# jkulhanek/viewformer

Measured on AMD Instinct MI355X. Metric: novel views/sec (encode->AR transformer->decode), 128px 6-ctx, higher is better.
Workload: dtype bf16

## Files before the change

viewformer_amd/csrc/gemm_bf16_g256.hip:

```cpp
#include "vf_common.h"
#include "epilogue.h"
#include "../../include/vf_hip.h"

namespace {

typedef __bf16 bf16x8 __attribute__((ext_vector_type(8)));
typedef __bf16 bf16x2_t __attribute__((ext_vector_type(2)));

constexpr int GM = 256, GN = 256, GK = 64;
constexpr int GA_BYTES = GM * GK * 2;
constexpr int GB_BYTES = GN * GK * 2;
constexpr int GSTAGE = GA_BYTES + GB_BYTES;

__device__ __forceinline__ void bufds16(__amdgpu_buffer_rsrc_t r, void* l, unsigned voff, unsigned soff) {
    __builtin_amdgcn_raw_ptr_buffer_load_lds(r, (__attribute__((address_space(3))) void*)l, 16, voff, soff, 0, 0);
}

template <bool DROP, int IC>
__device__ __forceinline__ void g256_store_f32(const vf_igemm_args& p, const f32x16 (&acc)[IC][2], int m_tile0, int n_tile0, int wrow0,
                                               int wave_n, int half, int l31, bool full, bool gelu) {
    const long long ldc = p.ldc, ldr = p.ldr;
    const bool has_res = p.res != nullptr;
    const bool dual = p.epilogue == VF_EPI_GELU_DUAL;
    const int odd = l31 & 1;
    const uint32_t drop_thresh = vf_dropout_thresh(p.drop_rate), drop_key = vf_dropout_key(p.drop_seed, p.drop_site, 0u);
    const float drop_scale = 1.0f / (1.0f - p.drop_rate);
#pragma unroll
    for (int j = 0; j < 2; ++j) {
        const int n = n_tile0 + wave_n * 64 + j * 32 + l31;
        const float bias = p.bias ? p.bias[n] : 0.f;
#pragma unroll
        for (int i = 0; i < IC; ++i) {
            int m0 = m_tile0 + wrow0 + i * 32 + 4 * half;
            if constexpr (DROP) asm volatile("" : "+v"(m0) :: "memory");
            const int rows_left = p.M - m0;
            float* o = p.out + (size_t)(rows_left > 0 ? m0 : 0) * ldc + n;
            float v[16];
#pragma unroll
            for (int r = 0; r < 16; ++r) v[r] = acc[i][j][r] + bias;
            if (gelu) {
#pragma unroll
                for (int r = 0; r < 16; ++r) v[r] = vf_gelu_erf_fast(v[r]);
            }
            if constexpr (DROP) {
#pragma unroll
                for (int g = 0; g < 4; ++g) {
                    const uint32_t w = vf_dropout_word(drop_key, (uint32_t)(((m0 + p.drop_row0) >> 2) + 2 * g) * (uint32_t)p.Cout + (uint32_t)n);
#pragma unroll
                    for (int e = 0; e < 4; ++e) v[4 * g + e] = vf_dropout_keep(w, e, drop_thresh) ? v[4 * g + e] * drop_scale : 0.f;
                }
            }
            if (has_res) {
                const float* rs = p.res + (size_t)(rows_left > 0 ? m0 : 0) * ldr + n;
                float rr[16];
#pragma unroll
                for (int r = 0; r < 16; ++r) {
                    const int row = (r & 3) + 8 * (r >> 2);
                    rr[r] = rs[(long long)(full || row < rows_left ? row : 0) * ldr];
                }
#pragma unroll
                for (int r = 0; r < 16; ++r) v[r] += rr[r];
            }
            if (full) {
#pragma unroll
                for (int r = 0; r < 16; ++r) o[(long long)((r & 3) + 8 * (r >> 2)) * ldc] = v[r];
            } else if (rows_left > 0) {
#pragma unroll
                for (int r = 0; r < 16; ++r) {
                    const int row = (r & 3) + 8 * (r >> 2);
                    if (row < rows_left) o[(long long)row * ldc] = v[r];
                }
            }
            if (dual) {
                __builtin_amdgcn_sched_barrier(0);
                __bf16* o16 = reinterpret_cast<__bf16*>(p.out_aux) + (size_t)(rows_left > 0 ? m0 : 0) * ldc + (n - odd);
#pragma unroll
                for (int r = 0; r < 16; ++r) v[r] = vf_gelu_erf_fast(v[r]);
#pragma unroll
                for (int r = 0; r < 16; r += 2) {
                    const float give = odd ? v[r] : v[r + 1];
                    const float got = vf_lane_xor1(give);
                    const int row = ((r + odd) & 3) + 8 * ((r + odd) >> 2);
                    bf16x2_t h;
                    h[0] = (__bf16)(odd ? got : v[r]);
                    h[1] = (__bf16)(odd ? v[r + 1] : got);
                    if (full || row < rows_left) *reinterpret_cast<bf16x2_t*>(o16 + (long long)row * ldc) = h;
                }
            }
            __builtin_amdgcn_sched_barrier(0);
        }
    }
}

template <int EPI, bool FULL, int IC>
__device__ __forceinline__ void g256_store_bf16(const vf_igemm_args& p, const f32x16 (&acc)[IC][2], int m_tile0, int n_tile0, int wrow0,
                                                int wave_n, int half, int l31) {
    __bf16* __restrict__ O = reinterpret_cast<__bf16*>(p.out);
    const int odd = l31 & 1;
#pragma unroll
    for (int j = 0; j < 2; ++j) {
        const int n = n_tile0 + wave_n * 64 + j * 32 + l31;
        const float bias = p.bias ? p.bias[n] : 0.f;
#pragma unroll
        for (int i = 0; i < IC; ++i) {
            const int m0 = m_tile0 + wrow0 + i * 32 + 4 * half;
            float t[16];
            if (EPI == 2 || EPI == 4) {
                const bool u16 = p.reserved0 & 4;
                const unsigned esz = u16 ? 2u : 4u;
                const __amdgpu_buffer_rsrc_t u_rs = __builtin_amdgcn_make_buffer_rsrc(
                    const_cast<unsigned char*>(reinterpret_cast<const unsigned char*>(p.res) + (size_t)m_tile0 * p.ldr * esz), 0,
                    (int)min((long long)0x7fffffff, (long long)(p.M - m_tile0) * p.ldr * esz), 0x00020000);
                float uu[16];
                if (u16) {
                    const unsigned voff = ((unsigned)(m0 - m_tile0) * (unsigned)p.ldr + (unsigned)(n - odd)) * 2u;
                    unsigned w[8];
#pragma unroll
                    for (int r = 0; r < 16; r += 2) {
                        const int row = ((r + odd) & 3) + 8 * ((r + odd) >> 2);
                        w[r >> 1] = __builtin_amdgcn_raw_buffer_load_b32(u_rs, voff + (unsigned)row * (unsigned)p.ldr * 2u, 0, 0);
                    }
#pragma unroll
                    for (int r = 0; r < 16; r += 2) {
                        const unsigned mine = w[r >> 1];
                        const unsigned give = odd ? (mine << 16) : (mine & 0xffff0000u);
                        const unsigned got = vf_lane_xor1(give);
                        uu[r] = __builtin_bit_cast(float, odd ? got : (mine << 16));
                        uu[r + 1] = __builtin_bit_cast(float, odd ? (mine & 0xffff0000u) : got);
                    }
                } else {
                    const unsigned voff = ((unsigned)(m0 - m_tile0) * (unsigned)p.ldr + (unsigned)n) * 4u;
#pragma unroll
                    for (int r = 0; r < 16; ++r) {
                        const unsigned soff = (unsigned)((r & 3) + 8 * (r >> 2)) * (unsigned)p.ldr * 4u;
                        uu[r] = __builtin_bit_cast(float, __builtin_amdgcn_raw_buffer_load_b32(u_rs, voff, soff, 0));
                    }
                }
                __builtin_amdgcn_sched_barrier(0);
#pragma unroll
                for (int q = 0; q < 4; ++q) {
#pragma unroll
                    for (int e = 0; e < 4; ++e)
                        t[4 * q + e] = __fmul_rn(__fadd_rn(acc[i][j][4 * q + e], bias), EPI == 4 ? uu[4 * q + e] : vf_gelu_grad_fast(uu[4 * q + e]));
                    __builtin_amdgcn_sched_barrier(0);
                }
            } else {
#pragma unroll
                for (int r = 0; r < 16; ++r) {
                    t[r] = acc[i][j][r] + bias;
                    if (EPI == 1) t[r] = vf_gelu_erf_fast(t[r]);
                }
            }
            float gq[EPI == 5 ? 16 : 1];
            if (EPI == 5) {
#pragma unroll
                for (int r = 0; r < 16; ++r) { float f, g; vf_gelu_and_grad_fast(t[r], f, g); t[r] = f; gq[r] = g; }
            }
#pragma unroll
            for (int pass = 0; pass < ((EPI == 3 || EPI == 5) ? 2 : 1); ++pass) {
                __bf16* __restrict__ dst = pass == 0 ? O : reinterpret_cast<__bf16*>(p.out_aux);
                if (EPI == 3 && pass == 1) {
                    __builtin_amdgcn_sched_barrier(0);
#pragma unroll
                    for (int r = 0; r < 16; ++r) t[r] = vf_gelu_erf_fast(t[r]);
                }
#pragma unroll
                for (int r = 0; r < 16; r += 2) {
                    const float lo = (EPI == 5 && pass == 0) ? gq[r] : t[r], hi = (EPI == 5 && pass == 0) ? gq[r + 1] : t[r + 1];
                    const float give = odd ? lo : hi;
                    const float got = vf_lane_xor1(give);
                    const int m = m0 + ((r + odd) & 3) + 8 * ((r + odd) >> 2);
                    bf16x2_t v;
                    v[0] = (__bf16)(odd ? got : lo);
                    v[1] = (__bf16)(odd ? hi : got);
                    if (FULL || m < p.M) *reinterpret_cast<bf16x2_t*>(dst + (size_t)m * p.ldc + (n - odd)) = v;
                }
            }
        }
    }
}

template <bool O16, bool DROP, int IC>
__device__ __forceinline__ void g256_tile(const vf_igemm_args& p, unsigned char* smem_b, int m_tile0, int nblk, int tid) {
    constexpr int TROWS = 2 * IC * 32;
    const int lane = tid & 63;
    const int wave = __builtin_amdgcn_readfirstlane(tid >> 6);
    const int wave_m = wave >> 2, wave_n = wave & 3;
    const int half = lane >> 5, l31 = lane & 31;
    const int wrow0 = wave_m * (IC * 32);
    const int n_tile0 = nblk * GN;
    const int nstages = p.Cin / GK;

    const bool a_mover = wave * 32 < TROWS;
    const __amdgpu_buffer_rsrc_t a_rsrc = __builtin_amdgcn_make_buffer_rsrc(const_cast<float*>(p.x), 0, 0x7fffffff, 0x00020000);
    const __amdgpu_buffer_rsrc_t w_rsrc = __builtin_amdgcn_make_buffer_rsrc(const_cast<float*>(p.w_packed), 0, 0x7fffffff, 0x00020000);
    unsigned avoff[4];
#pragma unroll
    for (int q = 0; q < 4; ++q) {
        const int r = wave * 32 + q * 8 + (lane >> 3);
        const int c = (lane & 7) ^ ((r >> 1) & 7);
        int m = m_tile0 + r;
        m = m < p.M ? m : p.M - 1;
        avoff[q] = (unsigned)(((size_t)m * p.lda) * 2 + c * 16);
    }
    const unsigned wvoff = (unsigned)((size_t)nblk * GB_BYTES + wave * 4096 + lane * 16);
    const size_t w_stage_stride = (size_t)(p.Cout / 128) * (GK * 128 * 2);
    auto issue = [&](int s) {
        unsigned char* dst = smem_b + (s & 1) * GSTAGE;
        if (IC == 4 || a_mover) {
#pragma unroll
            for (int q = 0; q < 4; ++q) bufds16(a_rsrc, dst + (wave * 32 + q * 8) * 128, avoff[q], (unsigned)(s * (GK * 2)));
        }
#pragma unroll
        for (int q = 0; q < 4; ++q) bufds16(w_rsrc, dst + GA_BYTES + wave * 4096 + q * 1024, wvoff + q * 1024, (unsigned)((size_t)s * w_stage_stride));
    };

    const unsigned a_row_off = (unsigned)((wrow0 + l31) * 128);
    const unsigned a_swz = (unsigned)((l31 >> 1) & 7);
    unsigned a_off[4];
#pragma unroll
    for (int ks = 0; ks < 4; ++ks) a_off[ks] = a_row_off + ((((unsigned)(ks * 2 + half)) ^ a_swz) << 4);
    const unsigned b_off = (unsigned)(GA_BYTES + (wave_n >> 1) * (GK * 128 * 2) + ((half * 128) + (wave_n & 1) * 64 + l31) * 16);

    f32x16 acc[IC][2];
#pragma unroll
    for (int i = 0; i < IC; ++i)
#pragma unroll
        for (int j = 0; j < 2; ++j)
#pragma unroll
            for (int r = 0; r < 16; ++r) acc[i][j][r] = 0.f;

    issue(0);
    for (int s = 0; s < nstages; ++s) {
        asm volatile("s_waitcnt vmcnt(0) lgkmcnt(0)" ::: "memory");
        __builtin_amdgcn_s_barrier();
        if (s + 1 < nstages) issue(s + 1);
        const unsigned char* buf = smem_b + (s & 1) * GSTAGE;
        bf16x8 a[2][IC], b[2][2];
        auto frags = [&](int ks, bf16x8 (&af)[IC], bf16x8 (&bf)[2]) {
#pragma unroll
            for (int j = 0; j < 2; ++j) bf[j] = *reinterpret_cast<const bf16x8*>(buf + b_off + (ks * 2 * 128 + j * 32) * 16);
#pragma unroll
            for (int i = 0; i < IC; ++i) af[i] = *reinterpret_cast<const bf16x8*>(buf + a_off[ks] + i * (32 * 128));
        };
        frags(0, a[0], b[0]);
#pragma unroll
        for (int ks = 0; ks < 4; ++ks) {
            if (ks < 3) frags(ks + 1, a[(ks + 1) & 1], b[(ks + 1) & 1]);
            __builtin_amdgcn_sched_barrier(0);
#pragma unroll
            for (int i = 0; i < IC; ++i)
#pragma unroll
                for (int j = 0; j < 2; ++j)
                    acc[i][j] = __builtin_amdgcn_mfma_f32_32x32x16_bf16(a[ks & 1][i], b[ks & 1][j], acc[i][j], 0, 0, 0);
            __builtin_amdgcn_sched_barrier(0);
        }
    }

    const bool full = m_tile0 + TROWS <= p.M;
    const bool gelu = p.epilogue == VF_EPI_GELU_ERF;
    if (O16) {
        const bool gbwd = p.epilogue == VF_EPI_GELU_BWD;
        const bool dual16 = p.epilogue == VF_EPI_GELU_DUAL;
        const bool deriv = p.reserved0 & 8;
        if (dual16 && deriv) {
            if (full) g256_store_bf16<5, true, IC>(p, acc, m_tile0, n_tile0, wrow0, wave_n, half, l31);
            else g256_store_bf16<5, false, IC>(p, acc, m_tile0, n_tile0, wrow0, wave_n, half, l31);
        } else if (gbwd && deriv) {
            if (full) g256_store_bf16<4, true, IC>(p, acc, m_tile0, n_tile0, wrow0, wave_n, half, l31);
            else g256_store_bf16<4, false, IC>(p, acc, m_tile0, n_tile0, wrow0, wave_n, half, l31);
        } else if (dual16) {
            if (full) g256_store_bf16<3, true, IC>(p, acc, m_tile0, n_tile0, wrow0, wave_n, half, l31);
            else g256_store_bf16<3, false, IC>(p, acc, m_tile0, n_tile0, wrow0, wave_n, half, l31);
        } else if (full) {
            if (gbwd) g256_store_bf16<2, true, IC>(p, acc, m_tile0, n_tile0, wrow0, wave_n, half, l31);
            else if (gelu) g256_store_bf16<1, true, IC>(p, acc, m_tile0, n_tile0, wrow0, wave_n, half, l31);
            else g256_store_bf16<0, true, IC>(p, acc, m_tile0, n_tile0, wrow0, wave_n, half, l31);
        } else {
            if (gbwd) g256_store_bf16<2, false, IC>(p, acc, m_tile0, n_tile0, wrow0, wave_n, half, l31);
            else if (gelu) g256_store_bf16<1, false, IC>(p, acc, m_tile0, n_tile0, wrow0, wave_n, half, l31);
            else g256_store_bf16<0, false, IC>(p, acc, m_tile0, n_tile0, wrow0, wave_n, half, l31);
        }
    } else {
        g256_store_f32<DROP, IC>(p, acc, m_tile0, n_tile0, wrow0, wave_n, half, l31, full, gelu);
    }
}

__device__ __forceinline__ void g256_panel_order(unsigned lbid, int mt, int nb, int& mtile, int& nblk) {
    constexpr int PANEL = 4;
    const int sn = nb <= PANEL ? nb : nb % PANEL == 0 ? PANEL : nb % 3 == 0 ? 3 : nb % 2 == 0 ? 2 : 1;
    const int per_panel = mt * sn;
    const int panel = (int)(lbid / (unsigned)per_panel);
    const int in_panel = (int)(lbid - (unsigned)panel * per_panel);
    nblk = panel * sn + in_panel % sn;
    mtile = in_panel / sn;
}

template <bool O16, bool DROP = false, bool TAIL = false>
__global__ __launch_bounds__(512, 1) void gemm_bf16_g256_kernel(vf_igemm_args p, int f_rows, int h_rows, int tail_ic) {
    extern __shared__ __attribute__((aligned(16))) unsigned char smem_b[];
    const int tid = threadIdx.x;
    const int nb = p.Cout / GN;
    int mtile, nblk;
    if constexpr (!TAIL) {
        g256_panel_order(vf_xcd_bid(), (p.M + GM - 1) / GM, nb, mtile, nblk);
        g256_tile<O16, DROP, 4>(p, smem_b, mtile * GM, nblk, tid);
    } else {
        const unsigned F = (unsigned)(f_rows * nb), tot = gridDim.x;
        const unsigned x = blockIdx.x & 7u, i = blockIdx.x >> 3;
        const unsigned nF = F / 8u + (x < (F & 7u) ? 1u : 0u);
        const unsigned baseF = x * (F / 8u) + (x < (F & 7u) ? x : (F & 7u));
        if (i < nF) {
            g256_panel_order(baseF + i, f_rows, nb, mtile, nblk);
            g256_tile<O16, DROP, 4>(p, smem_b, mtile * GM, nblk, tid);
            return;
        }
        const unsigned baseT = x * (tot / 8u) + (x < (tot & 7u) ? x : (tot & 7u));
        g256_panel_order(baseT - baseF + (i - nF), h_rows, nb, mtile, nblk);
        const int m_tile0 = f_rows * GM + mtile * (tail_ic * 64);
        if (tail_ic == 3) g256_tile<O16, DROP, 3>(p, smem_b, m_tile0, nblk, tid);
        else g256_tile<O16, DROP, 2>(p, smem_b, m_tile0, nblk, tid);
    }
}

}

struct G256Tail { int f_rows, h_rows, ic; };
static G256Tail g256_tail_policy(int M, int nb) {
    const int mt = (M + GM - 1) / GM;
    const long long ntiles = (long long)mt * nb;
    constexpr int CUS = 256;
    G256Tail none{0, 0, 0};
    if (ntiles <= CUS || !vf_selected(VF_SEL_GEMM_TAIL)) return none;
    const int last = (int)(ntiles % CUS);
    if (last == 0 || last > (CUS * 3) / 4 - 8 || last < 16) return none;
    const int f_rows = (int)((ntiles / CUS) * CUS / nb);
    if (f_rows <= 0 || f_rows >= mt) return none;
    const int rem_blocks = (M - f_rows * GM + 31) / 32;
    for (int ic = 2; ic <= 3; ++ic) {
        const int h_rows = (rem_blocks + 2 * ic - 1) / (2 * ic);
        if ((long long)h_rows * nb <= CUS) return G256Tail{f_rows, h_rows, ic};
    }
    return none;
}

int vf_gemm_bf16_g256_launch(const vf_igemm_args& a, hipStream_t stream) {
    const bool a16 = a.reserved0 & 1, o16 = a.reserved0 & 2;
    if (!a16 || a.batch > 1 || a.Cout % GN != 0 || a.Cin % GK != 0 || a.M < GM || (a.lda & 7)) return VF_ERR_UNSUPPORTED;
    if (o16 && ((a.res && a.epilogue != VF_EPI_GELU_BWD) || (a.ldc & 1))) return VF_ERR_UNSUPPORTED;
    if (a.epilogue == VF_EPI_GELU_BWD && !(o16 && a.res)) return VF_ERR_UNSUPPORTED;
    if (a.epilogue == VF_EPI_GELU_DUAL && (a.res || !a.out_aux || (a.ldc & 1))) return VF_ERR_UNSUPPORTED;
    if ((a.reserved0 & 4) && a.epilogue != VF_EPI_GELU_BWD) return VF_ERR_BAD_ARG;
    if (a.reserved0 & 8) {
        if (a.epilogue == VF_EPI_GELU_BWD ? !(a.reserved0 & 4) : !(a.epilogue == VF_EPI_GELU_DUAL && o16)) return VF_ERR_BAD_ARG;
    }
    if (a.res && a.epilogue == VF_EPI_GELU_ERF) return VF_ERR_UNSUPPORTED;
    if (a.drop_rate != 0.f && (!(a.drop_rate > 0.f && a.drop_rate < 1.f) || o16 || a.epilogue != VF_EPI_NONE || a.drop_row0 < 0 || (a.drop_row0 & 3) ||
                               (((unsigned long long)a.M + (unsigned long long)a.drop_row0 + 3) / 4) * (unsigned long long)a.Cout >= (1ull << 32)))
        return VF_ERR_UNSUPPORTED;
    if ((size_t)a.M * a.lda * 2 >= (1ull << 31) || (size_t)a.Cin * a.Cout * 2 >= (1ull << 31)) return VF_ERR_UNSUPPORTED;
    const int mt = (a.M + GM - 1) / GM, nb = a.Cout / GN;
    const G256Tail t = g256_tail_policy(a.M, nb);
    const dim3 g((unsigned)(t.f_rows ? (t.f_rows + t.h_rows) * nb : mt * nb));
    auto launch = [&](auto kernel, unsigned long long* devs) -> int {
        if (vf_attr_needed(devs)) {
            const hipError_t e = hipFuncSetAttribute(reinterpret_cast<const void*>(kernel), hipFuncAttributeMaxDynamicSharedMemorySize, 2 * GSTAGE);
            if (e != hipSuccess) return (int)e;
            vf_attr_done(devs);
        }
        hipLaunchKernelGGL(kernel, g, dim3(512), (size_t)2 * GSTAGE, stream, a, t.f_rows, t.h_rows, t.ic);
        return vf_last_status();
    };
    static unsigned long long d0 = 0, d1 = 0, d2 = 0, d3 = 0, d4 = 0, d5 = 0;
    const bool drop = a.drop_rate > 0.f;
    if (t.f_rows) {
        if (o16) return launch(gemm_bf16_g256_kernel<true, false, true>, &d3);
        return drop ? launch(gemm_bf16_g256_kernel<false, true, true>, &d5) : launch(gemm_bf16_g256_kernel<false, false, true>, &d4);
    }
    if (o16) return launch(gemm_bf16_g256_kernel<true, false, false>, &d0);
    return drop ? launch(gemm_bf16_g256_kernel<false, true, false>, &d2) : launch(gemm_bf16_g256_kernel<false, false, false>, &d1);
}
```

Before: 1142.

## Add phased ping-pong K-loop with split half-tile loads for 256x256 GEMM

Adds a new main loop for the full 256x256 tile that breaks each K-tile into four quarter-tile MFMA phases. Loads for the next stages are issued at fine granularity between phases, with explicit waitcnt and barriers, and s_setprio raises MFMA priority. The two wave_m halves are staggered by an extra barrier so that one group's math overlaps the other's LDS reads and global-to-LDS copies. The goal is to hide load latency that the old full-stage wait-then-compute loop exposed, at the cost of more barriers and delicate waitcnt accounting. It is used whenever Cin/64 is even and at least 4.

```diff
diff --git a/viewformer_amd/csrc/gemm_bf16_g256.hip b/viewformer_amd/csrc/gemm_bf16_g256.hip
--- a/viewformer_amd/csrc/gemm_bf16_g256.hip
+++ b/viewformer_amd/csrc/gemm_bf16_g256.hip
@@ -180,8 +180,114 @@
     }
 }
 
-template <bool O16, bool DROP, int IC>
+__device__ __forceinline__ void g256_loop_phased(const vf_igemm_args& p, unsigned char* smem_b, int m_tile0, int nblk, int wave, int lane,
+                                                 f32x16 (&acc)[4][2]) {
+    const int wave_m = wave >> 2, wave_n = wave & 3;
+    const int half = lane >> 5, l31 = lane & 31;
+    const int nkt = p.Cin / GK;
+    const __amdgpu_buffer_rsrc_t a_rsrc = __builtin_amdgcn_make_buffer_rsrc(const_cast<float*>(p.x), 0, 0x7fffffff, 0x00020000);
+    const __amdgpu_buffer_rsrc_t w_rsrc = __builtin_amdgcn_make_buffer_rsrc(const_cast<float*>(p.w_packed), 0, 0x7fffffff, 0x00020000);
+    unsigned a_src[2][2], w_src[2][2];
+    int a_dst[2][2], w_dst[2][2];
+#pragma unroll
+    for (int h = 0; h < 2; ++h)
+#pragma unroll
+        for (int q = 0; q < 2; ++q) {
+            const int pc = wave * 2 + q;
+            const int r0 = (pc >> 3) * 128 + h * 64 + (pc & 7) * 8;
+            const int r = r0 + (lane >> 3);
+            const int c = (lane & 7) ^ ((r >> 1) & 7);
+            int m = m_tile0 + r;
+            m = m < p.M ? m : p.M - 1;
+            a_src[h][q] = (unsigned)(((size_t)m * p.lda) * 2 + c * 16);
+            a_dst[h][q] = r0 * 128;
+            const int wn = pc >> 2, ks = pc & 3;
+            w_src[h][q] = (unsigned)((size_t)nblk * GB_BYTES + (wn >> 1) * (GK * 128 * 2) + ks * 4096 + half * 2048 + ((wn & 1) * 64 + h * 32 + l31) * 16);
+            w_dst[h][q] = GA_BYTES + h * 16384 + pc * 1024;
+        }
+    const unsigned w_stage_stride = (unsigned)((size_t)(p.Cout / 128) * (GK * 128 * 2));
+    auto stage_a = [&](int h, int par, int t) {
+#pragma unroll
+        for (int q = 0; q < 2; ++q) bufds16(a_rsrc, smem_b + par * GSTAGE + a_dst[h][q], a_src[h][q], (unsigned)(t * (GK * 2)));
+    };
+    auto stage_b = [&](int j, int par, int t) {
+#pragma unroll
+        for (int q = 0; q < 2; ++q) bufds16(w_rsrc, smem_b + par * GSTAGE + w_dst[j][q], w_src[j][q], (unsigned)t * w_stage_stride);
+    };
+    const unsigned a_swz = (unsigned)((l31 >> 1) & 7);
+    unsigned a_off[4];
+#pragma unroll
+    for (int ks = 0; ks < 4; ++ks) a_off[ks] = (unsigned)((wave_m * 128 + l31) * 128) + ((((unsigned)(ks * 2 + half)) ^ a_swz) << 4);
+    const unsigned b_off = (unsigned)(GA_BYTES + wave_n * 4096 + half * 512 + l31 * 16);
+    auto rd_a = [&](const unsigned char* buf, int ih, bf16x8 (&af)[2][4]) {
+#pragma unroll
+        for (int ks = 0; ks < 4; ++ks)
+#pragma unroll
+            for (int ii = 0; ii < 2; ++ii) af[ii][ks] = *reinterpret_cast<const bf16x8*>(buf + a_off[ks] + (2 * ih + ii) * (32 * 128));
+    };
+    auto rd_b = [&](const unsigned char* buf, int j, bf16x8 (&bf)[4]) {
+#pragma unroll
+        for (int ks = 0; ks < 4; ++ks) bf[ks] = *reinterpret_cast<const bf16x8*>(buf + b_off + j * 16384 + ks * 1024);
+    };
+    auto mma = [&](int ih, int j, const bf16x8 (&af)[2][4], const bf16x8 (&bf)[4]) {
+        __builtin_amdgcn_s_barrier();
+        asm volatile("s_waitcnt lgkmcnt(0)" ::: "memory");
+        __builtin_amdgcn_sched_barrier(0);
+        __builtin_amdgcn_s_setprio(1);
+#pragma unroll
+        for (int ks = 0; ks < 4; ++ks)
+#pragma unroll
+            for (int ii = 0; ii < 2; ++ii)
+                acc[2 * ih + ii][j] = __builtin_amdgcn_mfma_f32_32x32x16_bf16(af[ii][ks], bf[ks], acc[2 * ih + ii][j], 0, 0, 0);
+        __builtin_amdgcn_s_setprio(0);
+        __builtin_amdgcn_sched_barrier(0);
+        __builtin_amdgcn_s_barrier();
+    };
+    auto ktile = [&](int par, int mode, int t) {
+        const unsigned char* buf = smem_b + par * GSTAGE;
+        bf16x8 a0[2][4], a1[2][4], b0[4], b1[4];
+        rd_b(buf, 0, b0);
+        __builtin_amdgcn_sched_barrier(0);
+        rd_a(buf, 0, a0);
+        __builtin_amdgcn_sched_barrier(0);
+        if (mode <= 1) stage_a(1, par ^ 1, t + 1);
+        asm volatile("s_waitcnt lgkmcnt(8)" ::: "memory");
+        mma(0, 0, a0, b0);
+
+        rd_b(buf, 1, b1);
+        if (mode == 0) stage_b(0, par, t + 2);
+        if (mode == 2) asm volatile("s_waitcnt vmcnt(0)" ::: "memory");
+        mma(0, 1, a0, b1);
+
+        rd_a(buf, 1, a1);
+        if (mode == 0) stage_a(0, par, t + 2);
+        mma(1, 1, a1, b1);
+
+        if (mode == 0) {
+            stage_b(1, par, t + 2);
+            asm volatile("s_waitcnt vmcnt(6)" ::: "memory");
+        }
+        if (mode == 1) asm volatile("s_waitcnt vmcnt(2)" ::: "memory");
+        mma(1, 0, a1, b0);
+    };
+
+    stage_a(0, 0, 0); stage_b(0, 0, 0); stage_b(1, 0, 0); stage_a(1, 0, 0);
+    stage_b(0, 1, 1); stage_a(0, 1, 1); stage_b(1, 1, 1);
+    asm volatile("s_waitcnt vmcnt(6)" ::: "memory");
+    __builtin_amdgcn_s_barrier();
+    if (wave_m == 1) __builtin_amdgcn_s_barrier();
+    for (int t = 0; t < nkt - 2; t += 2) {
+        ktile(0, 0, t);
+        ktile(1, 0, t + 1);
+    }
+    ktile(0, 1, nkt - 2);
+    ktile(1, 2, nkt - 1);
+    if (wave_m == 0) __builtin_amdgcn_s_barrier();
+}
+
+template <bool O16, bool DROP, int IC, bool PHASED = false>
 __device__ __forceinline__ void g256_tile(const vf_igemm_args& p, unsigned char* smem_b, int m_tile0, int nblk, int tid) {
+    static_assert(!PHASED || IC == 4, "the phased loop is the full tile's");
     constexpr int TROWS = 2 * IC * 32;
     const int lane = tid & 63;
     const int wave = __builtin_amdgcn_readfirstlane(tid >> 6);
@@ -189,8 +295,19 @@
     const int half = lane >> 5, l31 = lane & 31;
     const int wrow0 = wave_m * (IC * 32);
     const int n_tile0 = nblk * GN;
+
+    f32x16 acc[IC][2];
+#pragma unroll
+    for (int i = 0; i < IC; ++i)
+#pragma unroll
+        for (int j = 0; j < 2; ++j)
+#pragma unroll
+            for (int r = 0; r < 16; ++r) acc[i][j][r] = 0.f;
+
+    if constexpr (PHASED) {
+        g256_loop_phased(p, smem_b, m_tile0, nblk, wave, lane, acc);
+    } else {
     const int nstages = p.Cin / GK;
-
     const bool a_mover = wave * 32 < TROWS;
     const __amdgpu_buffer_rsrc_t a_rsrc = __builtin_amdgcn_make_buffer_rsrc(const_cast<float*>(p.x), 0, 0x7fffffff, 0x00020000);
     const __amdgpu_buffer_rsrc_t w_rsrc = __builtin_amdgcn_make_buffer_rsrc(const_cast<float*>(p.w_packed), 0, 0x7fffffff, 0x00020000);
@@ -221,14 +338,6 @@
 #pragma unroll
     for (int ks = 0; ks < 4; ++ks) a_off[ks] = a_row_off + ((((unsigned)(ks * 2 + half)) ^ a_swz) << 4);
     const unsigned b_off = (unsigned)(GA_BYTES + (wave_n >> 1) * (GK * 128 * 2) + ((half * 128) + (wave_n & 1) * 64 + l31) * 16);
-
-    f32x16 acc[IC][2];
-#pragma unroll
-    for (int i = 0; i < IC; ++i)
-#pragma unroll
-        for (int j = 0; j < 2; ++j)
-#pragma unroll
-            for (int r = 0; r < 16; ++r) acc[i][j][r] = 0.f;
 
     issue(0);
     for (int s = 0; s < nstages; ++s) {
@@ -255,6 +364,7 @@
                     acc[i][j] = __builtin_amdgcn_mfma_f32_32x32x16_bf16(a[ks & 1][i], b[ks & 1][j], acc[i][j], 0, 0, 0);
             __builtin_amdgcn_sched_barrier(0);
         }
+    }
     }
 
     const bool full = m_tile0 + TROWS <= p.M;
@@ -296,7 +406,7 @@
     mtile = in_panel / sn;
 }
 
-template <bool O16, bool DROP = false, bool TAIL = false>
+template <bool O16, bool DROP = false, bool TAIL = false, bool PHASED = false>
 __global__ __launch_bounds__(512, 1) void gemm_bf16_g256_kernel(vf_igemm_args p, int f_rows, int h_rows, int tail_ic) {
     extern __shared__ __attribute__((aligned(16))) unsigned char smem_b[];
     const int tid = threadIdx.x;
@@ -304,7 +414,7 @@
     int mtile, nblk;
     if constexpr (!TAIL) {
         g256_panel_order(vf_xcd_bid(), (p.M + GM - 1) / GM, nb, mtile, nblk);
-        g256_tile<O16, DROP, 4>(p, smem_b, mtile * GM, nblk, tid);
+        g256_tile<O16, DROP, 4, PHASED>(p, smem_b, mtile * GM, nblk, tid);
     } else {
         const unsigned F = (unsigned)(f_rows * nb), tot = gridDim.x;
         const unsigned x = blockIdx.x & 7u, i = blockIdx.x >> 3;
@@ -312,7 +422,7 @@
         const unsigned baseF = x * (F / 8u) + (x < (F & 7u) ? x : (F & 7u));
         if (i < nF) {
             g256_panel_order(baseF + i, f_rows, nb, mtile, nblk);
-            g256_tile<O16, DROP, 4>(p, smem_b, mtile * GM, nblk, tid);
+            g256_tile<O16, DROP, 4, PHASED>(p, smem_b, mtile * GM, nblk, tid);
             return;
         }
         const unsigned baseT = x * (tot / 8u) + (x < (tot & 7u) ? x : (tot & 7u));
@@ -372,7 +482,17 @@
         return vf_last_status();
     };
     static unsigned long long d0 = 0, d1 = 0, d2 = 0, d3 = 0, d4 = 0, d5 = 0;
+    static unsigned long long e0 = 0, e1 = 0, e2 = 0, e3 = 0, e4 = 0, e5 = 0;
     const bool drop = a.drop_rate > 0.f;
+    const int nkt = a.Cin / GK;
+    if (nkt >= 4 && nkt % 2 == 0) {
+        if (t.f_rows) {
+            if (o16) return launch(gemm_bf16_g256_kernel<true, false, true, true>, &e3);
+            return drop ? launch(gemm_bf16_g256_kernel<false, true, true, true>, &e5) : launch(gemm_bf16_g256_kernel<false, false, true, true>, &e4);
+        }
+        if (o16) return launch(gemm_bf16_g256_kernel<true, false, false, true>, &e0);
+        return drop ? launch(gemm_bf16_g256_kernel<false, true, false, true>, &e2) : launch(gemm_bf16_g256_kernel<false, false, false, true>, &e1);
+    }
     if (t.f_rows) {
         if (o16) return launch(gemm_bf16_g256_kernel<true, false, true>, &d3);
         return drop ? launch(gemm_bf16_g256_kernel<false, true, true>, &d5) : launch(gemm_bf16_g256_kernel<false, false, true>, &d4);
```

Result: no change. 1146 (median of 6 runs) (+0.4%).
